# lanterndata/lantern

Hardware: AMD Instinct MI355X
Metric: QPS (recall@10 alongside), 1000000x768 f32 l2sq ef=64 k=10 (higher is better)
Workload: dtype f32

## Files before the change

include/lantern_gpu.h:

```cpp
#ifndef LANTERN_GPU_H
#define LANTERN_GPU_H

#include <stdbool.h>
#include <stddef.h>
#include <stdint.h>

#ifdef __cplusplus
extern "C" {
#endif

#define LANTERN_GPU_EXPORT __attribute__((visibility("default")))


typedef void       *usearch_index_t;
typedef uint64_t    usearch_key_t;
typedef uint64_t    usearch_label_t;
typedef float       usearch_distance_t;
typedef const char *usearch_error_t;

typedef enum usearch_metric_kind_t {
    usearch_metric_unknown_k = 0,
    usearch_metric_cos_k = 1,
    usearch_metric_l2sq_k = 3,
    usearch_metric_hamming_k = 8
// ... 186 lines not shown
LANTERN_GPU_EXPORT void lantern_gpu_last_filtered_each(usearch_index_t, uint32_t out[6], usearch_error_t *);
LANTERN_GPU_EXPORT void lantern_gpu_set_search_shape(usearch_index_t, int waves_per_query, int max_workgroups,
                                                     usearch_error_t *);

LANTERN_GPU_EXPORT void lantern_gpu_exact_search(usearch_index_t, const void *queries, size_t nq, size_t k,
                                                 uint32_t *slots, float *distances, usearch_error_t *);

LANTERN_GPU_EXPORT size_t lantern_gpu_dense_profile(int on, float *ms, uint32_t *rows, uint32_t *cols, uint32_t *fused, size_t cap);
LANTERN_GPU_EXPORT void lantern_gpu_exact_knn_stats(uint64_t *queries, uint64_t *certified, uint64_t *fallback);

LANTERN_GPU_EXPORT void lantern_gpu_search_row_trace(usearch_index_t, int on, size_t nq, size_t per_query_cap, uint32_t *trace,
                                                     uint32_t *counts, usearch_error_t *);

LANTERN_GPU_EXPORT int lantern_gpu_last_search_grid(usearch_index_t, usearch_error_t *);
LANTERN_GPU_EXPORT const char *lantern_gpu_plan_search(const int64_t in[31], uint32_t out[12]);

LANTERN_GPU_EXPORT void lantern_gpu_distance_gather(usearch_index_t, const void *query, const uint32_t *slots,
                                                    size_t n, float *out, usearch_error_t *);
LANTERN_GPU_EXPORT float lantern_gpu_last_gather_ms(usearch_index_t, usearch_error_t *);
LANTERN_GPU_EXPORT void lantern_gpu_search_screen_stats(usearch_index_t, uint64_t *logical, uint64_t *exact, usearch_error_t *);
LANTERN_GPU_EXPORT size_t lantern_gpu_export_screen(usearch_index_t, size_t first, size_t count, int8_t *rows, float *meta, float *norms,
                                                    usearch_error_t *);
LANTERN_GPU_EXPORT void lantern_gpu_screen_probe(usearch_index_t, const void *query, const uint32_t *slots, size_t n, float radius,
                                                 int workgroup, uint8_t *rejected, usearch_error_t *);
LANTERN_GPU_EXPORT void lantern_gpu_distance_matrix(const void *a, size_t na, const void *b, size_t nb,
                                                    usearch_scalar_kind_t, size_t dims, usearch_metric_kind_t,
                                                    int exact_order, float *out, usearch_error_t *);

LANTERN_GPU_EXPORT void lantern_gpu_assign_to_clusters(const float *dataset, size_t n, size_t row_dims, size_t subvector_start,
                                                       size_t subvector_dim, const float *centers, size_t k,
// ... 168 lines not shown
```

lantern_amd/capi.py:

```python
from __future__ import annotations

import ctypes as C
import os

import numpy as np

HERE = os.path.dirname(os.path.abspath(__file__))
LIB_PATH = os.path.join(HERE, "lib", "liblantern_gpu.so")

METRIC_COS, METRIC_L2SQ, METRIC_HAMMING = 1, 3, 8
SCALAR_F32, SCALAR_F16, SCALAR_I8, SCALAR_B1 = 1, 3, 4, 5
METRICS = {"cos": METRIC_COS, "l2sq": METRIC_L2SQ, "hamming": METRIC_HAMMING}
EMPTY = 0xFFFFFFFF
USEARCH_HEADER_SIZE = 136


class LanternGpuError(RuntimeError):
    pass


class InitOptions(C.Structure):
    _fields_ = [
        ("metric_kind", C.c_int),
        ("metric", C.c_void_p),
# ... 53 lines not shown
    "lantern_gpu_version", "lantern_gpu_device_count",
    "lantern_gpu_set_seed", "lantern_gpu_set_add_batch", "lantern_gpu_add_many", "lantern_gpu_flush",
    "lantern_gpu_add_with_level", "lantern_gpu_search_batch", "lantern_gpu_search_batch_device", "lantern_gpu_search_batch_device_strided",
    "lantern_gpu_set_search_shape", "lantern_gpu_exact_search", "lantern_gpu_dense_profile", "lantern_gpu_exact_knn_stats", "lantern_gpu_distance_gather",
    "lantern_gpu_host_alloc", "lantern_gpu_host_free", "lantern_gpu_save_stream", "lantern_gpu_pq_compact", "lantern_gpu_pq_expand", "lantern_gpu_memory_usage", "lantern_gpu_spec_profile", "lantern_gpu_search_unique_rows", "lantern_gpu_search_row_trace", "lantern_gpu_last_search_grid", "lantern_gpu_last_gather_ms", "lantern_gpu_search_screen_stats",
    "lantern_gpu_distance_matrix", "lantern_gpu_assign_to_clusters", "lantern_gpu_graph_info_get", "lantern_gpu_export_graph", "lantern_gpu_import_graph",
    "lantern_gpu_export_codes",
    "lantern_gpu_counters_get", "lantern_gpu_set_profiling", "lantern_gpu_build_profile_get", "lantern_gpu_search_phase_profile", "lantern_scan_begin", "lantern_scan_rescan", "lantern_scan_gettuple", "lantern_scan_trace", "lantern_scan_end",
    "lantern_l2sq_dist", "lantern_cos_dist", "lantern_hamming_dist", "lantern_index_server_start", "lantern_index_server_start_tls",
    "lantern_index_server_port", "lantern_index_server_status_port", "lantern_index_server_status",
    "lantern_index_server_served", "lantern_index_server_stop",
    "lantern_gpu_graph_checksum", "lantern_gpu_comm_unique_id", "lantern_gpu_comm_init_rccl", "lantern_gpu_comm_init_host",
    "lantern_gpu_comm_init_local", "lantern_gpu_comm_free", "lantern_gpu_comm_rank", "lantern_gpu_comm_world",
    "lantern_gpu_comm_set_timeout", "lantern_gpu_comm_stats", "lantern_gpu_comm_allgatherv_host",
    "lantern_gpu_comm_allgatherv_device", "lantern_gpu_shard_range", "lantern_gpu_add_sharded", "lantern_gpu_add_row_sharded", "lantern_gpu_search_partitioned", "lantern_gpu_search_batch_lane", "lantern_gpu_search_batch_lane_notify", "lantern_gpu_row_bytes",
    "lantern_gpu_level_for", "lantern_gpu_plan_batch", "lantern_gpu_row_shard_plan", "lantern_gpu_plan_search",
    "lantern_scan_server_start", "lantern_scan_server_start_fn", "lantern_scan_server_port", "lantern_scan_server_stats",
    "lantern_scan_server_batch_histogram", "lantern_scan_server_timing", "lantern_scan_server_stop", "lantern_scan_client_connect", "lantern_scan_client_search", "lantern_scan_client_search_next",
    "lantern_scan_client_close", "lantern_scan_begin_client",
    "lantern_mirror_acquire", "lantern_mirror_index", "lantern_mirror_version", "lantern_mirror_rebind", "lantern_mirror_advance", "lantern_mirror_release",
    "lantern_mirror_invalidate", "lantern_mirror_set_capacity", "lantern_mirror_stats",
    "UsearchNodeBytes", "usearch_init_node", "node_tuple_size", "label_from_node", "level_from_node", "reset_node_label", "get_node_neighbors_mut",
    "lantern_quant_bits_scalar_kind",
    "lantern_gpu_filter_from_labels", "lantern_gpu_filter_from_slot_bitmap", "lantern_gpu_filter_count", "lantern_gpu_filter_free",
    "lantern_gpu_set_filter_policy", "lantern_gpu_filter_stats", "lantern_gpu_last_filtered_launch", "lantern_gpu_search_batch_filtered", "lantern_gpu_search_batch_filtered_device",
    "lantern_gpu_cursor_search_filtered", "lantern_scan_set_filter",
    "lantern_gpu_filter_resident_bytes", "lantern_scan_server_start_filtered_fn", "lantern_scan_server_filter_stats", "lantern_scan_client_set_filter",
    "lantern_scan_client_clear_filter",
    "lantern_gpu_search_batch_filtered_each", "lantern_gpu_search_batch_filtered_each_device", "lantern_gpu_search_batch_filtered_each_lane", "lantern_gpu_last_filtered_each",
    "lantern_gpu_set_filter_seeds", "lantern_gpu_last_filtered_seeds",
    "lantern_gpu_search_batch_params", "lantern_gpu_search_batch_params_lane", "lantern_gpu_search_batch_params_lane_notify",
# ... 131 lines not shown
        "lantern_gpu_comm_world": (i32, [vp]),
        "lantern_gpu_comm_set_timeout": (None, [vp, C.c_double]),
        "lantern_gpu_comm_stats": (None, [vp, C.POINTER(u64), C.POINTER(u64)]),
        "lantern_gpu_comm_allgatherv_host": (None, [vp, vp, C.POINTER(sz), C.POINTER(sz), err]),
        "lantern_gpu_comm_allgatherv_device": (None, [vp, vp, C.POINTER(sz), C.POINTER(sz), vp, err]),
        "lantern_gpu_shard_range": (None, [sz, i32, i32, C.POINTER(sz), C.POINTER(sz)]),
        "lantern_gpu_add_sharded": (None, [vp, vp, vp, vp, sz, i32, err]),
        "lantern_gpu_add_row_sharded": (None, [vp, vp, vp, vp, sz, i32, err]),
        "lantern_gpu_search_partitioned": (None, [vp, vp, vp, sz, i32, sz, sz, vp, vp, vp, err]),
        "lantern_gpu_row_bytes": (sz, [vp, err]),
        "lantern_gpu_search_batch_lane": (None, [vp, i32, vp, sz, i32, sz, sz, vp, vp, vp, err]),
        "lantern_gpu_search_batch_lane_notify": (None, [vp, i32, vp, sz, i32, sz, sz, vp, vp, vp, vp, vp, err]),
        "lantern_gpu_level_for": (i32, [u64, u64, u32]),
        "lantern_gpu_plan_batch": (sz, [sz, i32, vp, sz, sz, sz]),
        "lantern_gpu_plan_search": (C.c_char_p, [vp, vp]),
        "lantern_gpu_row_shard_plan": (sz, [vp, i32, u64, u32, sz, sz, vp, vp, vp, sz]),
        "lantern_scan_server_start": (vp, [vp, C.c_char_p, i32, sz, C.c_uint, err]),
        "lantern_scan_server_start_fn": (vp, [BATCH_SEARCH_FN, vp, sz, C.c_char_p, i32, sz, C.c_uint, err]),
        "lantern_scan_server_port": (i32, [vp]),
        "lantern_scan_server_stats": (None, [vp, C.POINTER(u64), C.POINTER(u64), C.POINTER(u64), C.POINTER(u64)]),
        "lantern_scan_server_batch_histogram": (sz, [vp, C.POINTER(u64), sz]),
        "lantern_scan_server_timing": (None, [vp, C.POINTER(C.c_double)]),
        "lantern_scan_server_stop": (None, [vp]),
        "lantern_scan_client_connect": (vp, [C.c_char_p, i32, err]),
        "lantern_scan_client_search": (sz, [vp, vp, sz, sz, sz, vp, vp, err]),
        "lantern_scan_client_search_next": (sz, [vp, vp, sz, sz, sz, vp, vp, err]),
        "lantern_scan_client_close": (None, [vp]),
        "lantern_scan_begin_client": (vp, [vp, sz, i32, i32, err]),
        "lantern_mirror_acquire": (vp, [u64, u64, C.POINTER(InitOptions), vp, vp, sz, err]),
        "lantern_mirror_index": (vp, [vp]),
# ... 781 lines not shown

def plan_batch(size: int, max_level: int, pending_levels, max_batch: int, min_ratio: int) -> int:
    lv = np.ascontiguousarray(pending_levels, dtype=np.int32)
    return int(lib().lantern_gpu_plan_batch(size, max_level, _ptr(lv), lv.size, max_batch, min_ratio))


PLAN_SEARCH_IN = ("chunks", "M", "M0", "mcode", "n", "ef_default", "num_cus", "pq_compact", "pqd_inv", "pq_S16", "search_vis_slots", "search_max_wg",
                  "phase_profile", "spec_profile", "nq", "k", "ef", "skip", "waves", "each", "max_expansion", "env_spec_set", "env_spec",
                  "env_adc_spec_set", "env_adc_spec", "env_pq_adc", "env_spec_waves", "env_lds_list", "env_wide_rows", "env_solo", "env_waves_per_cu")
PLAN_SEARCH_OUT = ("path", "spec", "expansion", "waves", "grid", "vis_slots", "lds", "spec_prefetch", "spec_cache", "wide_rows", "took_spec", "lds_list")


def plan_search(fields) -> tuple[dict, str | None]:
    vals = [fields[n] for n in PLAN_SEARCH_IN] if isinstance(fields, dict) else list(fields)
    assert len(vals) == len(PLAN_SEARCH_IN)
    a, out = np.asarray(vals, dtype=np.int64), np.zeros(len(PLAN_SEARCH_OUT), dtype=np.uint32)
    why = lib().lantern_gpu_plan_search(_ptr(a), _ptr(out))
    return dict(zip(PLAN_SEARCH_OUT, (int(x) for x in out))), (why.decode() if why else None)


def row_shard_plan(shard_sizes, seed: int, M: int, max_batch: int, min_ratio: int):
    sizes = np.ascontiguousarray(shard_sizes, dtype=np.uint64)
    world = int(sizes.size)
    n = int(lib().lantern_gpu_row_shard_plan(_ptr(sizes), world, seed, M, max_batch, min_ratio, None, None, None, 0))
    first, count = np.zeros(max(n, 1), dtype=np.uintp), np.zeros(max(n, 1), dtype=np.uintp)
    share = np.zeros((max(n, 1), world), dtype=np.uintp)
    lib().lantern_gpu_row_shard_plan(_ptr(sizes), world, seed, M, max_batch, min_ratio, _ptr(first), _ptr(count), _ptr(share), n)
    return [(int(first[t]), int(count[t]), [int(x) for x in share[t]]) for t in range(n)]


def shard_range(n: int, world: int, rank: int) -> tuple[int, int]:
    b, e = C.c_size_t(), C.c_size_t()
    lib().lantern_gpu_shard_range(n, world, rank, C.byref(b), C.byref(e))
# ... 363 lines not shown
```

lantern_amd/csrc/device_common.hpp:

```cpp
#pragma once
#include <hip/hip_runtime.h>
#include <stdint.h>

namespace lgpu {

constexpr uint32_t EMPTY = 0xFFFFFFFFu;
#ifndef LGPU_ROW_BLOCK
#define LGPU_ROW_BLOCK 3
#endif
#ifndef LGPU_ROW_BLOCK_COS
#define LGPU_ROW_BLOCK_COS 2
#endif
#ifndef LGPU_LIST_PREFETCH
#define LGPU_LIST_PREFETCH 1
#endif
#ifndef LGPU_ROW_BLOCK1
#define LGPU_ROW_BLOCK1 4
#endif
#ifndef LGPU_SCREEN
#define LGPU_SCREEN 1
#endif

constexpr int M_COS = 1;
constexpr int M_L2SQ = 3;
// ... 480 lines not shown
    int32_t         max_level;
    const uint4    *pq_centers;
    uint32_t        pq_cps;
    uint32_t        pq_C;
    uint32_t        pq_inv;
    uint32_t        pq_row_bytes;
    const uint4    *screen;
    const float2   *screen_meta;
    uint32_t        screen_chunks;
};

__host__ __device__ __forceinline__ float screen_val(float s, uint32_t w, int b) { return s * (float)(int)(int8_t)(uint8_t)(w >> (8 * b)); }
__host__ __device__ inline bool screen_rows_for(uint32_t chunks) { return chunks >= 128; }
__host__ __device__ inline bool screen_cos_norm_ok(float r) { return r >= 0x1p-48f && r <= 0x1p48f; }
__host__ __device__ inline uint32_t screen_chunks_for(uint32_t chunks) { return (chunks + 3) / 4; }

__device__ __forceinline__ const uint4 *row_of(const View &v, uint32_t slot) { return v.vec + (size_t)slot * v.chunks; }

struct PqdRow
{
    const uint8_t *codes;
    const uint4   *centers;
    uint32_t       cps, C, inv;
    __device__ __forceinline__ uint4 operator[](int ch) const
    {
        const uint32_t sv = ((uint32_t)ch * inv) >> 16, off = (uint32_t)ch - sv * cps;
        const uint32_t code = codes[ sv ];
        return centers[ ((size_t)sv * C + code) * cps + off ];
    }
};
// ... 23 lines not shown
```

lantern_amd/csrc/index.hpp:

```cpp
#pragma once
#include <hip/hip_runtime.h>

#include <deque>
#include <mutex>
#include <string>
#include <thread>
#include <unordered_map>
#include <unordered_set>
#include <functional>
#include <vector>

#include "../../include/lantern_gpu.h"
#include "kernels.hpp"

namespace lgpu {

struct Cursor
{
    std::unordered_set<uint32_t> seen;
};

constexpr int kIndexLanes = 8;

enum ScratchSlot : int
// ... 199 lines not shown
uint32_t    vis_undo_cap();
int         search_grid(const Index *ix, size_t nq, int waves, int waves_per_cu);
int         search_grid(int num_cus, int max_wg, int forced_waves_per_cu, size_t nq, int waves, int waves_per_cu);
struct SearchEnv
{
    bool spec_set = false, adc_spec_set = false;
    int  spec = 0, spec_waves = 0, wide_rows = -1, waves_per_cu = 0;
    bool adc_spec = false, pq_adc = false, lds_list = false, solo = false;
};
SearchEnv search_env();
struct SearchPlanIn
{
    uint32_t  chunks = 0, M = 0, M0 = 0, ef_default = 0, pqd_inv = 0, pq_S16 = 0;
    int       mcode = 0, num_cus = 0, search_vis_slots = -1, search_max_wg = 0;
    bool      pq_compact = false, phase_profile = false, spec_profile = false;
    size_t    n = 0, nq = 0, k = 0, ef = 0, skip = 0;
    int       waves = 0;
    bool      each = false;
    uint32_t  max_expansion = 0;
    SearchEnv env;
};
enum SearchPath : uint32_t { kSearchAdc, kSearchPqd, kSearchClassic, kSearchSpec1, kSearchSpec2, kSearchTwin, kSearchSolo };
struct SearchPlan
{
    SearchPath  path = kSearchClassic;
    int         spec = 0, waves = 0, grid = 0, wide_rows = 0, lds_list = 0;
    uint32_t    expansion = 0, vis_slots = 0, spec_prefetch = 0, spec_cache = 0;
    size_t      lds = 0;
    bool        took_spec = false;
    const char *refusal = nullptr;
};
SearchPlan   plan_search(const SearchPlanIn &in);
SearchPlanIn search_plan_in(const Index *ix, size_t nq, size_t k, size_t ef, size_t skip, int waves);
struct EachLaunch
{
    const char *h_table = nullptr;
    size_t      table_bytes = 0;
    const char *d_table = nullptr;
    size_t      list_at = 0;
};
bool        run_search_device(Index *ix, const uint4 *d_queries, size_t nq, size_t k, size_t ef, size_t skip, const SearchOut &out,
                              hipStream_t stream, int waves, uint32_t *done = nullptr, uint32_t *done_flags = nullptr);
std::string params_check(const lantern_gpu_query_params *params, size_t nq, size_t k_stride);
// ... 30 lines not shown
```

lantern_amd/csrc/screen_probe_kernel.hip:

```cpp
#include "query_frame.hpp"

namespace lgpu {

constexpr uint32_t kProbeSlots = 64;

template <int METRIC>
__global__ void __launch_bounds__(512) k_screen_probe(View v, const uint4 *query, const uint32_t *slots, uint32_t n, float radius, uint8_t *out)
{
    constexpr int G = 64;
    const int     tid = threadIdx.x, T = blockDim.x;
    WalkLds       s;
    (void)carve_walk(lgpu_smem, s, v.chunks, kProbeSlots, kProbeSlots);
    if(tid == 0) {
        uint64_t *const sp = (uint64_t *)&s.scal[ S_SCREEN ];
        sp[ 0 ] = (uint64_t)v.screen;
        sp[ 1 ] = (uint64_t)v.screen_meta;
        s.scal[ S_NREJ ] = 0;
        s.scal[ S_NSURV ] = 0;
        s.scal[ S_QN2 ] = 0;
    }
    for(uint32_t i = tid; i < n; i += T) {
        s.newids[ i ] = slots[ i ];
        s.newkeys[ i ] = 0;
    }
    frame_stage<METRIC, G>(tid, T, s, query, 0, v.chunks);
    const float qn2 = __int_as_float(s.scal[ S_QN2 ]);
    (void)hop_distances_screened<METRIC, G, 2>(v, s, (int)n, make_key(radius, 0u), qn2);
    for(uint32_t i = tid; i < n; i += T) out[ i ] = s.newkeys[ i ] == ~0ull ? 1 : 0;
}

hipError_t launch_screen_probe(int metric, const View &v, const uint4 *query, const uint32_t *slots, uint32_t n, float radius, int threads,
                               uint8_t *out, hipStream_t stream)
{
    if(n == 0) return hipSuccess;
    if(n > kProbeSlots || (threads != 256 && threads != 512) || !v.screen || !v.screen_meta || !screen_rows_for(v.chunks)) return hipErrorInvalidValue;
    const size_t lds = walk_lds_bytes(v.chunks, kProbeSlots, kProbeSlots);
    if(metric == M_L2SQ) hipLaunchKernelGGL(k_screen_probe<M_L2SQ>, dim3(1), dim3(threads), lds, stream, v, query, slots, n, radius, out);
    else if(metric == M_COS) hipLaunchKernelGGL(k_screen_probe<M_COS>, dim3(1), dim3(threads), lds, stream, v, query, slots, n, radius, out);
    else return hipErrorInvalidValue;
    return hipGetLastError();
}

}
```

lantern_amd/csrc/search_kernel.hpp:

```cpp
#pragma once
#include <algorithm>
#include <cstddef>
#include <cstdlib>

#include "kernels.hpp"
#include "walk.hpp"
#include "walk_spec.hpp"
#ifndef LGPU_EXPERIMENTAL
#define LGPU_EXPERIMENTAL 0
#endif
#if LGPU_EXPERIMENTAL
#include "experimental/walk_twin.hpp"
#endif
#include "dispatch.hpp"
#include "query_frame.hpp"

namespace lgpu {

#define LGPU_SEARCH_ARG(base, field) LGPU_KARG(base, decltype(SearchArgs::field), offsetof(SearchArgs, field))
#define LGPU_VIEW_ARG(base, STRUCT, field) LGPU_KARG(base, decltype(View::field), offsetof(STRUCT, view) + offsetof(View, field))
#define LGPU_LOAD_VIEW(v, base, STRUCT)             \
    {                                               \
        v.vec = LGPU_VIEW_ARG(base, STRUCT, vec);   \
        v.chunks = LGPU_VIEW_ARG(base, STRUCT, chunks); \
// ... 59 lines not shown
            View               v;
            LGPU_LOAD_VIEW(v, ka, SearchArgs)
            if constexpr(METRIC >= M_PQD) LGPU_LOAD_VIEW_PQD(v, ka, SearchArgs)
            if constexpr(SCREEN) {
                if(tid == 0) {
                    uint64_t *const sp = (uint64_t *)&s.scal[ S_SCREEN ];
                    sp[ 0 ] = (uint64_t)LGPU_VIEW_ARG(ka, SearchArgs, screen);
                    sp[ 1 ] = (uint64_t)LGPU_VIEW_ARG(ka, SearchArgs, screen_meta);
                    s.scal[ S_NREJ ] = 0;
                }
            }
            uint32_t        bm_words;
            uint32_t *const bitmap = frame_bind<SearchArgs>(ka, s, bm_words);
            const int       ef = EACH ? (int)each.ef : (int)LGPU_SEARCH_ARG(ka, ef);
            frame_stage<METRIC, G>(tid, T, s, LGPU_FRAME_ARG(ka, SearchArgs, queries), q, v.chunks);
            if constexpr(PROF) {
                t_q = (unsigned long long)clock64();
                s.touched = LGPU_SEARCH_ARG(ka, touched);
                s.trace_cap = LGPU_SEARCH_ARG(ka, trace_cap);
                uint32_t *const tr = LGPU_SEARCH_ARG(ka, trace);
                s.trace = tr ? tr + (size_t)q * s.trace_cap : nullptr;
                s.trace_count = tr ? LGPU_SEARCH_ARG(ka, trace_count) + q : nullptr;
            }
            if(v.n != 0 && (!EACH || each.k != 0)) {
                uint32_t start;
                if constexpr(SPEC != 0) start = greedy_descent_spec<METRIC, G>(v, s, v.entry, v.max_level, 0, D);
                else start = greedy_descent<METRIC, G, PROF>(v, s, v.entry, v.max_level, 0, D);
                if constexpr(PROF) pc[ 6 ] = (unsigned long long)clock64() - t_q;
#if LGPU_EXPERIMENTAL
                if constexpr(SPEC == 3)
// ... 29 lines not shown
```

lantern_amd/csrc/search_launch.hpp:

```cpp
#pragma once
#include "search_kernel.hpp"

namespace lgpu {

#define LGPU_LAUNCH_SEARCH(...)                                                                                        \
    {                                                                                                                  \
        static LdsAttrCache attr_;        \
        ensure_dynamic_lds((const void *)k_search<__VA_ARGS__>, lds, attr_);    \
        hipLaunchKernelGGL((k_search<__VA_ARGS__>), dim3(grid), dim3(64 * waves), lds, stream, a);                     \
    }
#define LGPU_LAUNCH_SEARCH_KPL(MM, GG, PP, RR)                           \
    {                                                                    \
        if(kpl == 1) LGPU_LAUNCH_SEARCH(MM, GG, PP, RR, 1, 0, EACH)      \
        else if(kpl == 2) LGPU_LAUNCH_SEARCH(MM, GG, PP, RR, 2, 0, EACH) \
        else LGPU_LAUNCH_SEARCH(MM, GG, PP, RR, 0, 0, EACH)              \
    }

template <bool EACH> static hipError_t launch_search_classic(int metric, const SearchArgs &a, int waves, int grid, hipStream_t stream)
{
    if(EACH && a.phase_cycles) return hipErrorInvalidValue;
    const size_t lds = search_lds_bytes(a.view.chunks, a.ef, a.view.M0, a.frame.vis_slots);
    const int    kpl = a.lds_list ? 0 : a.ef <= 64 ? 1 : a.ef <= 128 ? 2 : 0;
    const int    G_ = group_lanes_for(a.view.chunks);
    if(a.wide_rows && !a.phase_cycles && G_ == 64) {
        bool launched = true;
        switch(metric) {
            case M_L2SQ: LGPU_LAUNCH_SEARCH_KPL(M_L2SQ, 64, false, 4); break;
            case M_COS: LGPU_LAUNCH_SEARCH_KPL(M_COS, 64, false, 4); break;
            case M_HAMMING: LGPU_LAUNCH_SEARCH_KPL(M_HAMMING, 64, false, 4); break;
            case M_L2SQ_F16: LGPU_LAUNCH_SEARCH_KPL(M_L2SQ_F16, 64, false, 4); break;
            case M_COS_F16: LGPU_LAUNCH_SEARCH_KPL(M_COS_F16, 64, false, 4); break;
            case M_L2SQ_PQD: LGPU_LAUNCH_SEARCH_KPL(M_L2SQ_PQD, 64, false, 4); break;
            case M_COS_PQD: LGPU_LAUNCH_SEARCH_KPL(M_COS_PQD, 64, false, 4); break;
            default: launched = false;
        }
        if(launched) return hipGetLastError();
// ... 72 lines not shown
```

lantern_amd/csrc/search_plan.cpp:

```cpp
#include "index.hpp"

#include <algorithm>
#include <cstdlib>
#include <cstring>

namespace lgpu {

SearchEnv search_env()
{
    SearchEnv e;
    if(const char *se = std::getenv("LANTERN_GPU_SPEC")) { e.spec_set = true; e.spec = std::atoi(se); }
    if(const char *se = std::getenv("LANTERN_GPU_ADC_SPEC")) { e.adc_spec_set = true; e.adc_spec = std::atoi(se) != 0; }
    if(const char *pa = std::getenv("LANTERN_GPU_PQ_ADC")) e.pq_adc = std::atoi(pa) != 0;
    if(const char *sw = std::getenv("LANTERN_GPU_SPEC_WAVES")) e.spec_waves = std::atoi(sw);
    if(const char *ll = std::getenv("LANTERN_GPU_LDS_LIST")) e.lds_list = std::atoi(ll) != 0;
    static const int  wide_env = std::getenv("LANTERN_GPU_WIDE_ROWS") ? std::atoi(std::getenv("LANTERN_GPU_WIDE_ROWS")) : -1;
    static const bool solo_auto = std::getenv("LANTERN_GPU_SOLO") && std::atoi(std::getenv("LANTERN_GPU_SOLO")) != 0;
    static const int  forced = std::getenv("LANTERN_GPU_WAVES_PER_CU") ? std::atoi(std::getenv("LANTERN_GPU_WAVES_PER_CU")) : 0;
    e.wide_rows = wide_env, e.solo = solo_auto, e.waves_per_cu = forced;
    return e;
}

SearchPlanIn search_plan_in(const Index *ix, size_t nq, size_t k, size_t ef, size_t skip, int waves)
{
    SearchPlanIn in;
    in.chunks = ix->chunks; in.M = ix->M; in.M0 = ix->M0; in.ef_default = ix->ef;
    in.mcode = ix->mcode; in.n = ix->n; in.num_cus = ix->num_cus;
    in.pq_compact = ix->pq_compact; in.pqd_inv = ix->pqd_inv; in.pq_S16 = ix->pq_S16;
    in.search_vis_slots = ix->search_vis_slots; in.search_max_wg = ix->search_max_wg;
    in.phase_profile = ix->phase_profile; in.spec_profile = ix->spec_profile;
    in.nq = nq; in.k = k; in.ef = ef; in.skip = skip; in.waves = waves;
    in.env = search_env();
    return in;
}

SearchPlan plan_search(const SearchPlanIn &in)
{
    const SearchEnv &env = in.env;
    const size_t     nq = in.nq;
    int              waves = in.waves;
    SearchPlan       p;
    size_t expansion = in.ef ? in.ef : in.ef_default;
    if(expansion < in.k + in.skip) expansion = in.k + in.skip;
    if(in.each) expansion = in.max_expansion;
    p.expansion = (uint32_t)expansion;
// ... 60 lines not shown
                    return p;
                }
            }
            if(spec == 3 && !(expansion <= 64 && (in.mcode == M_L2SQ || in.mcode == M_COS) && (group_lanes_for(in.chunks) == 64 || (in.mcode == M_L2SQ && group_lanes_for(in.chunks) == 16))))
                spec = 2;
#endif
        }
        waves = spec >= 2 ? 11 : spec == 1 ? 4 : waves < 0 ? -waves : 4;
        if(spec && env.spec_waves >= (spec >= 2 ? 4 : 2) && env.spec_waves <= (spec >= 2 ? 11 : 8)) waves = env.spec_waves;
    }
    const int      G_ = group_lanes_for(in.chunks), LW_ = G_ >= 32 ? 1 : G_ == 16 ? 2 : 4;
    const uint32_t spec_prefetch = spec && in.M0 % (uint32_t)LW_ == 0 && in.M0 <= (uint32_t)(G_ * LW_) ? 1u : 0u;
    const uint32_t spec_cache = !spec_prefetch ? 0u : spec >= 2 ? 128u : 64u;
    const size_t   spec_lds = spec ? search_spec_lds_bytes(in.M0, spec_prefetch, spec_cache, spec == 3) : 0;
    const size_t lds_budget = spec >= 2 ? 96 * 1024 : spec == 1 ? 39 * 1024 : 26 * 1024;
    uint32_t vis_slots = 1024;
    while(vis_slots < 8192 && vis_slots / 4 * 3 < expansion * in.M0 * 2) vis_slots <<= 1;
    if(in.search_vis_slots >= 0) vis_slots = (uint32_t)in.search_vis_slots / 4 * 4;
    while(vis_slots && search_lds_bytes(in.chunks, (uint32_t)expansion, in.M0, vis_slots) + spec_lds > lds_budget)
        vis_slots = vis_slots > 256 ? vis_slots - 256 : 0;
    if(vis_slots && vis_slots < 4 * in.M0) vis_slots = 0;
    p.lds = search_lds_bytes(in.chunks, (uint32_t)expansion, in.M0, vis_slots) + spec_lds;
    if(p.lds > 160 * 1024) { p.refusal = "lantern_gpu: ef/k exceed the 160 KiB LDS budget of the search kernel"; return p; }
    p.path = pqd ? kSearchPqd : spec == 0 ? kSearchClassic : spec == 1 ? kSearchSpec1 : spec == 2 ? kSearchSpec2 : kSearchTwin;
    p.spec = spec, p.took_spec = spec != 0;
    p.waves = waves, p.grid = search_grid(in.num_cus, in.search_max_wg, env.waves_per_cu, nq, waves, spec >= 2 ? waves : spec == 1 ? 16 : 24);
    p.vis_slots = vis_slots, p.spec_prefetch = spec_prefetch, p.spec_cache = spec_cache;
    p.wide_rows = spec ? 0 : env.wide_rows >= 0 ? env.wide_rows : (nq * (size_t)waves <= (size_t)in.num_cus * 16 && nq >= 64);
    return p;
}

static bool search_launch(Index *ix, const SearchPlan &p, const uint4 *d_queries, size_t nq, size_t k, size_t skip, const SearchOut &out,
                          hipStream_t stream, uint32_t *done, uint32_t *done_flags, const EachLaunch *each)
{
    const bool adc = p.path == kSearchAdc, pqd = p.path == kSearchPqd, solo = p.path == kSearchSolo;
    ix->last_search_grid = p.grid;
    const int slot = acquire_search_slot(ix, stream, (size_t)p.grid);
// ... 2 lines not shown
    a.view = ix->view();
    a.frame.queries = d_queries;
    a.frame.nq = (uint32_t)nq, a.k = (uint32_t)k, a.ef = p.expansion, a.skip = (uint32_t)skip;
    a.frame.labels = ix->d_labels;
    a.frame.out_labels = out.labels, a.frame.out_dists = out.dists, a.frame.out_slots = out.slots;
    a.frame.out_counts = out.counts, a.frame.out_D = out.D, a.frame.out_E = out.E;
    if(!solo) a.frame.bitmaps = ix->slot_bitmaps[ slot ], a.frame.bm_words = (uint32_t)ix->slot_words[ slot ], a.frame.undo_cap = vis_undo_cap();
    a.frame.vis_slots = p.vis_slots;
    a.frame.totals = ix->d_totals;
    a.screen_totals = ix->d_screen ? ix->d_totals + 48 : nullptr;
    a.frame.ticket = next_ticket(ix, nq, p.grid, stream);
    a.done = done, a.done_flags = done_flags;
    a.lds_list = p.lds_list, a.wide_rows = p.wide_rows;
    a.spec = p.spec, a.spec_prefetch = p.spec_prefetch, a.spec_cache = p.spec_cache;
    hipError_t e = hipSuccess;
    if(adc || pqd) a.view.vec = (const uint4 *)ix->d_codes16;
    if(adc) {
        a.view.chunks = ix->pq_S16 / 16;
        a.adc_centers = ix->d_centers;
        a.adc_S = ix->pq_S, a.adc_C = ix->pq_C, a.adc_subdim = ix->pq_subdim, a.adc_qchunks = ix->chunks;
    } else {
        if(pqd) {
            a.view.pq_centers = (const uint4 *)ix->d_centers;
            a.view.pq_cps = ix->pq_subdim / 4;
            a.view.pq_C = ix->pq_C;
            a.view.pq_inv = ix->pqd_inv;
            a.view.pq_row_bytes = ix->pq_S16;
        }
        const bool prof_walk = ix->phase_profile && !pqd && !each;
        a.phase_cycles = each ? nullptr : p.spec ? (ix->spec_profile ? ix->d_totals + 16 : nullptr) : prof_walk ? ix->d_totals + 8 : nullptr;
// ... 96 lines not shown
        at += cls[ c ].size();
    }
    for(int c = 0; c < 3; ++c) {
        if(cls[ c ].empty()) continue;
        if(!search_launch(ix, plans[ c ], d_queries, cls[ c ].size(), k_stride, 0, out, stream, nullptr, done_flags, &each[ c ])) return false;
        launches += 1;
        any_spec |= plans[ c ].took_spec ? 1u : 0u;
    }
    const uint32_t shape[ 6 ] = { launches, (uint32_t)cls[ 0 ].size(), (uint32_t)cls[ 1 ].size(), (uint32_t)cls[ 2 ].size(), std::max(top[ 0 ], std::max(top[ 1 ], top[ 2 ])), any_spec };
    std::copy(std::begin(shape), std::end(shape), ix->last_params);
    return true;
}

}

extern "C" const char *lantern_gpu_plan_search(const int64_t in[ 31 ], uint32_t out[ 12 ])
{
    if(!in || !out) return "lantern_gpu: null array";
    lgpu::SearchPlanIn s;
    s.chunks = (uint32_t)in[ 0 ]; s.M = (uint32_t)in[ 1 ]; s.M0 = (uint32_t)in[ 2 ]; s.mcode = (int)in[ 3 ]; s.n = (size_t)in[ 4 ];
    s.ef_default = (uint32_t)in[ 5 ]; s.num_cus = (int)in[ 6 ]; s.pq_compact = in[ 7 ] != 0; s.pqd_inv = (uint32_t)in[ 8 ]; s.pq_S16 = (uint32_t)in[ 9 ];
    s.search_vis_slots = (int)in[ 10 ]; s.search_max_wg = (int)in[ 11 ]; s.phase_profile = in[ 12 ] != 0; s.spec_profile = in[ 13 ] != 0;
    s.nq = (size_t)in[ 14 ]; s.k = (size_t)in[ 15 ]; s.ef = (size_t)in[ 16 ]; s.skip = (size_t)in[ 17 ]; s.waves = (int)in[ 18 ];
    s.each = in[ 19 ] != 0; s.max_expansion = (uint32_t)in[ 20 ];
    s.env.spec_set = in[ 21 ] != 0; s.env.spec = (int)in[ 22 ]; s.env.adc_spec_set = in[ 23 ] != 0; s.env.adc_spec = in[ 24 ] != 0;
    s.env.pq_adc = in[ 25 ] != 0; s.env.spec_waves = (int)in[ 26 ]; s.env.lds_list = in[ 27 ] != 0; s.env.wide_rows = (int)in[ 28 ];
    s.env.solo = in[ 29 ] != 0; s.env.waves_per_cu = (int)in[ 30 ];
    const lgpu::SearchPlan p = lgpu::plan_search(s);
    const uint32_t flat[ 12 ] = { (uint32_t)p.path, (uint32_t)p.spec, p.expansion, (uint32_t)p.waves, (uint32_t)p.grid, p.vis_slots, (uint32_t)p.lds,
                                  p.spec_prefetch, p.spec_cache, (uint32_t)p.wide_rows, p.took_spec ? 1u : 0u, (uint32_t)p.lds_list };
    std::copy(std::begin(flat), std::end(flat), out);
    return p.refusal;
}
```

lantern_amd/csrc/walk.hpp:

```cpp
#pragma once
#include <type_traits>

#include "device_common.hpp"

namespace lgpu {

enum { S_POS = 0, S_NNEW, S_CNT, S_ANY, S_BAD, S_CUR, S_CURD, S_CHANGED, S_VISCNT, S_SPILL, S_QN2, S_NNEW0, S_NNEW1, S_ANY0, S_ANY1,
       S_FRONT = 16, S_WORST = 20,
       S_MASK = 24,
       S_SCALARS = 28,
       S_NSURV = S_ANY0, S_NREJ = S_ANY1, S_SCREEN = S_MASK };

struct WalkLds
{
    uint4    *q;
    uint64_t *keys;
    uint64_t *keys2;
    uint64_t *newkeys;
    uint64_t *sorted;
    uint32_t *newids;
    int      *scal;
    uint32_t *vis;
    uint32_t  vis_slots;
    uint32_t *touched;
// ... 317 lines not shown
        if(gl == G - 1) {
            reread();
            uint64_t k0 = make_key(d0, id0);
            s.newkeys[ at(i) ] = k0;
            bool any = k0 < worst;
            if(j < nnew) {
                uint64_t k1 = make_key(d1, id1);
                s.newkeys[ at(j) ] = k1;
                any |= k1 < worst;
            }
            if(ANY && any) *any_slot = 1;
        }
    }
}

template <int METRIC, int G, int ROWS>
__device__ __forceinline__ int hop_distances_screened(const View &v, WalkLds &s, int nnew, uint64_t worst, float qn2)
{
    static_assert(METRIC == M_L2SQ || METRIC == M_COS, "the screen serves the f32 l2sq and cosine walks");
    constexpr int GS = 8, NB = 3;
    static_assert(G % GS == 0, "a screen group lies within one wave");
    const int       tid = threadIdx.x, T = blockDim.x, gs = tid / GS, gsl = tid % GS, NGS = T / GS;
    uint32_t *const surv = (uint32_t *)s.sorted;
    typedef uint32_t u32x4 __attribute__((ext_vector_type(4)));
    typedef float    f32x2 __attribute__((ext_vector_type(2)));
    typedef const __attribute__((address_space(1))) u32x4 *ScreenRow;
    typedef const __attribute__((address_space(1))) f32x2 *ScreenMeta;
    auto uniform = [](uint64_t x) {
        return (uint64_t)(uint32_t)__builtin_amdgcn_readfirstlane((int)(uint32_t)x) |
               (uint64_t)(uint32_t)__builtin_amdgcn_readfirstlane((int)(uint32_t)(x >> 32)) << 32;
    };
    const ScreenRow  screen = (ScreenRow)uniform(((const uint64_t *)&s.scal[ S_SCREEN ])[ 0 ]);
    const ScreenMeta screen_meta = (ScreenMeta)uniform(((const uint64_t *)&s.scal[ S_SCREEN ])[ 1 ]);
    const uint32_t   chunks = v.chunks, sch = screen_chunks_for(chunks);
    for(int j = gs; j < nnew; j += NGS) {
        const uint32_t id = s.newids[ j ];
        const ScreenRow row = screen + (size_t)id * sch;
        const f32x2     meta = screen_meta[ id ];
        float          acc = 0.f;
        for(uint32_t base = (uint32_t)gsl; base < sch; base += NB * GS) {
            u32x4 y[ NB ];
#pragma unroll
            for(int c = 0; c < NB; ++c)
                if(base + c * GS < sch) y[ c ] = row[ base + c * GS ];
#pragma unroll
            for(int c = 0; c < NB; ++c)
                if(base + c * GS < sch) {
                    const uint32_t w[ 4 ] = { y[ c ].x, y[ c ].y, y[ c ].z, y[ c ].w };
#pragma unroll
                    for(int k = 0; k < 4; ++k) {
                        const uint32_t qc = 4 * (base + c * GS) + (uint32_t)k;
                        const uint4    x = qc < chunks ? s.q[ qc ] : make_uint4(0u, 0u, 0u, 0u);
                        const float    xs[ 4 ] = { __uint_as_float(x.x), __uint_as_float(x.y), __uint_as_float(x.z), __uint_as_float(x.w) };
#pragma unroll
                        for(int b = 0; b < 4; ++b) {
                            if constexpr(METRIC == M_COS) {
                                acc = __builtin_fmaf(xs[ b ], (float)(int)(int8_t)(uint8_t)(w[ k ] >> (8 * b)), acc);
                            } else {
                                const float t = xs[ b ] - screen_val(meta.x, w[ k ], b);
                                acc = __builtin_fmaf(t, t, acc);
                            }
                        }
                    }
                }
        }
        acc = group_sum<GS>(acc);
        if(gsl == GS - 1) {
            bool reject = false;
            if constexpr(METRIC == M_COS) {
                const float rd = key_dist(worst), e = fmaxf(0x1p-12f, (float)(2 * chunks + 64) * 0x1p-24f);
                if(screen_cos_norm_ok(qn2)) {
                    const float sim8 = (acc * meta.x) / qn2;
                    const float ub = (sim8 + meta.y) + e;
                    reject = (1.f - ub) - e > rd;
                }
            } else {
                const float rd = key_dist(worst), ome = 1.f - fmaxf(0x1p-12f, (float)(2 * chunks + 64) * 0x1p-24f);
                if(__builtin_isfinite(acc)) {
                    const float a = __builtin_sqrtf(acc) * ome - meta.y;
                    const float lb = a > 0.f ? a * a : 0.f;
                    reject = lb > 0x1p-100f && lb * ome > rd;
                }
            }
            if(reject) s.newkeys[ j ] = ~0ull;
            else surv[ atomicAdd(&s.scal[ S_NSURV ], 1) ] = (uint32_t)j;
        }
    }
    __syncthreads();
    const int ns = s.scal[ S_NSURV ];
    if(tid == 0) s.scal[ S_NREJ ] += nnew - ns;
    return ns;
}

template <int METRIC, int G, bool PROF = false, int ROWS = 2>
__device__ int search_level(const View &v, WalkLds &s, uint32_t *bitmap, uint32_t bm_words, uint32_t start, int level, int ef,
                            uint32_t &D, uint32_t &E, unsigned long long *prof = nullptr)
// ... 434 lines not shown
```

Baseline: 2.297 million.

## Quantize query to int16 planes for integer dot4 screen distance bounds

The f32 query is quantized once per search into hi/lo int8 planes stored in extra LDS, together with a scale, an error bound and the quantized norm. The int8 screen pass then computes the distance bound with integer dot4 instructions instead of per-byte float FMAs, widening the bound by the quantization error so it stays conservative. The search planner reserves the extra LDS, which can shrink the visited-slot table, and it turns screening off for configurations it does not support.

```diff
diff --git a/include/lantern_gpu.h b/include/lantern_gpu.h
--- a/include/lantern_gpu.h
+++ b/include/lantern_gpu.h
@@ -224,6 +224,7 @@
 
 LANTERN_GPU_EXPORT int lantern_gpu_last_search_grid(usearch_index_t, usearch_error_t *);
 LANTERN_GPU_EXPORT const char *lantern_gpu_plan_search(const int64_t in[31], uint32_t out[12]);
+LANTERN_GPU_EXPORT const char *lantern_gpu_plan_search_screen(const int64_t in[32], uint32_t out[13]);
 
 LANTERN_GPU_EXPORT void lantern_gpu_distance_gather(usearch_index_t, const void *query, const uint32_t *slots,
                                                     size_t n, float *out, usearch_error_t *);
diff --git a/lantern_amd/capi.py b/lantern_amd/capi.py
--- a/lantern_amd/capi.py
+++ b/lantern_amd/capi.py
@@ -91,7 +91,7 @@
     "lantern_gpu_comm_init_local", "lantern_gpu_comm_free", "lantern_gpu_comm_rank", "lantern_gpu_comm_world",
     "lantern_gpu_comm_set_timeout", "lantern_gpu_comm_stats", "lantern_gpu_comm_allgatherv_host",
     "lantern_gpu_comm_allgatherv_device", "lantern_gpu_shard_range", "lantern_gpu_add_sharded", "lantern_gpu_add_row_sharded", "lantern_gpu_search_partitioned", "lantern_gpu_search_batch_lane", "lantern_gpu_search_batch_lane_notify", "lantern_gpu_row_bytes",
-    "lantern_gpu_level_for", "lantern_gpu_plan_batch", "lantern_gpu_row_shard_plan", "lantern_gpu_plan_search",
+    "lantern_gpu_level_for", "lantern_gpu_plan_batch", "lantern_gpu_row_shard_plan", "lantern_gpu_plan_search", "lantern_gpu_plan_search_screen",
     "lantern_scan_server_start", "lantern_scan_server_start_fn", "lantern_scan_server_port", "lantern_scan_server_stats",
     "lantern_scan_server_batch_histogram", "lantern_scan_server_timing", "lantern_scan_server_stop", "lantern_scan_client_connect", "lantern_scan_client_search", "lantern_scan_client_search_next",
     "lantern_scan_client_close", "lantern_scan_begin_client",
@@ -253,6 +253,7 @@
         "lantern_gpu_level_for": (i32, [u64, u64, u32]),
         "lantern_gpu_plan_batch": (sz, [sz, i32, vp, sz, sz, sz]),
         "lantern_gpu_plan_search": (C.c_char_p, [vp, vp]),
+        "lantern_gpu_plan_search_screen": (C.c_char_p, [vp, vp]),
         "lantern_gpu_row_shard_plan": (sz, [vp, i32, u64, u32, sz, sz, vp, vp, vp, sz]),
         "lantern_scan_server_start": (vp, [vp, C.c_char_p, i32, sz, C.c_uint, err]),
         "lantern_scan_server_start_fn": (vp, [BATCH_SEARCH_FN, vp, sz, C.c_char_p, i32, sz, C.c_uint, err]),
@@ -1064,9 +1065,15 @@
 def plan_search(fields) -> tuple[dict, str | None]:
     vals = [fields[n] for n in PLAN_SEARCH_IN] if isinstance(fields, dict) else list(fields)
     assert len(vals) == len(PLAN_SEARCH_IN)
-    a, out = np.asarray(vals, dtype=np.int64), np.zeros(len(PLAN_SEARCH_OUT), dtype=np.uint32)
-    why = lib().lantern_gpu_plan_search(_ptr(a), _ptr(out))
-    return dict(zip(PLAN_SEARCH_OUT, (int(x) for x in out))), (why.decode() if why else None)
+    if isinstance(fields, dict) and "screen" in fields:
+        names = PLAN_SEARCH_OUT + ("screen_lds",)
+        a, out = np.asarray(vals + [fields["screen"]], dtype=np.int64), np.zeros(len(names), dtype=np.uint32)
+        why = lib().lantern_gpu_plan_search_screen(_ptr(a), _ptr(out))
+    else:
+        names = PLAN_SEARCH_OUT
+        a, out = np.asarray(vals, dtype=np.int64), np.zeros(len(names), dtype=np.uint32)
+        why = lib().lantern_gpu_plan_search(_ptr(a), _ptr(out))
+    return dict(zip(names, (int(x) for x in out))), (why.decode() if why else None)
 
 
 def row_shard_plan(shard_sizes, seed: int, M: int, max_batch: int, min_ratio: int):
diff --git a/lantern_amd/csrc/device_common.hpp b/lantern_amd/csrc/device_common.hpp
--- a/lantern_amd/csrc/device_common.hpp
+++ b/lantern_amd/csrc/device_common.hpp
@@ -518,6 +518,8 @@
 __host__ __device__ inline bool screen_rows_for(uint32_t chunks) { return chunks >= 128; }
 __host__ __device__ inline bool screen_cos_norm_ok(float r) { return r >= 0x1p-48f && r <= 0x1p48f; }
 __host__ __device__ inline uint32_t screen_chunks_for(uint32_t chunks) { return (chunks + 3) / 4; }
+__host__ __device__ inline uint32_t screen_query_lds_bytes(uint32_t chunks) { return 16 + screen_chunks_for(chunks) * 32; }
+__host__ __device__ inline bool screen_l2_scale_ok(float s) { return s >= 0x1p-40f && s <= 0x1p40f; }
 
 __device__ __forceinline__ const uint4 *row_of(const View &v, uint32_t slot) { return v.vec + (size_t)slot * v.chunks; }
 
diff --git a/lantern_amd/csrc/index.hpp b/lantern_amd/csrc/index.hpp
--- a/lantern_amd/csrc/index.hpp
+++ b/lantern_amd/csrc/index.hpp
@@ -237,6 +237,7 @@
     uint32_t  chunks = 0, M = 0, M0 = 0, ef_default = 0, pqd_inv = 0, pq_S16 = 0;
     int       mcode = 0, num_cus = 0, search_vis_slots = -1, search_max_wg = 0;
     bool      pq_compact = false, phase_profile = false, spec_profile = false;
+    bool      screen = false;
     size_t    n = 0, nq = 0, k = 0, ef = 0, skip = 0;
     int       waves = 0;
     bool      each = false;
@@ -250,6 +251,7 @@
     int         spec = 0, waves = 0, grid = 0, wide_rows = 0, lds_list = 0;
     uint32_t    expansion = 0, vis_slots = 0, spec_prefetch = 0, spec_cache = 0;
     size_t      lds = 0;
+    uint32_t    screen_lds = 0;
     bool        took_spec = false;
     const char *refusal = nullptr;
 };
diff --git a/lantern_amd/csrc/screen_probe_kernel.hip b/lantern_amd/csrc/screen_probe_kernel.hip
--- a/lantern_amd/csrc/screen_probe_kernel.hip
+++ b/lantern_amd/csrc/screen_probe_kernel.hip
@@ -25,6 +25,7 @@
     }
     frame_stage<METRIC, G>(tid, T, s, query, 0, v.chunks);
     const float qn2 = __int_as_float(s.scal[ S_QN2 ]);
+    screen_stage_query<METRIC>(tid, s, v.chunks, qn2);
     (void)hop_distances_screened<METRIC, G, 2>(v, s, (int)n, make_key(radius, 0u), qn2);
     for(uint32_t i = tid; i < n; i += T) out[ i ] = s.newkeys[ i ] == ~0ull ? 1 : 0;
 }
@@ -34,7 +35,7 @@
 {
     if(n == 0) return hipSuccess;
     if(n > kProbeSlots || (threads != 256 && threads != 512) || !v.screen || !v.screen_meta || !screen_rows_for(v.chunks)) return hipErrorInvalidValue;
-    const size_t lds = walk_lds_bytes(v.chunks, kProbeSlots, kProbeSlots);
+    const size_t lds = walk_lds_bytes(v.chunks, kProbeSlots, kProbeSlots) + screen_query_lds_bytes(v.chunks);
     if(metric == M_L2SQ) hipLaunchKernelGGL(k_screen_probe<M_L2SQ>, dim3(1), dim3(threads), lds, stream, v, query, slots, n, radius, out);
     else if(metric == M_COS) hipLaunchKernelGGL(k_screen_probe<M_COS>, dim3(1), dim3(threads), lds, stream, v, query, slots, n, radius, out);
     else return hipErrorInvalidValue;
diff --git a/lantern_amd/csrc/search_kernel.hpp b/lantern_amd/csrc/search_kernel.hpp
--- a/lantern_amd/csrc/search_kernel.hpp
+++ b/lantern_amd/csrc/search_kernel.hpp
@@ -97,6 +97,9 @@
             uint32_t *const bitmap = frame_bind<SearchArgs>(ka, s, bm_words);
             const int       ef = EACH ? (int)each.ef : (int)LGPU_SEARCH_ARG(ka, ef);
             frame_stage<METRIC, G>(tid, T, s, LGPU_FRAME_ARG(ka, SearchArgs, queries), q, v.chunks);
+            if constexpr(SCREEN) {
+                if(LGPU_VIEW_ARG(ka, SearchArgs, screen)) screen_stage_query<METRIC>(tid, s, v.chunks, __int_as_float(s.scal[ S_QN2 ]));
+            }
             if constexpr(PROF) {
                 t_q = (unsigned long long)clock64();
                 s.touched = LGPU_SEARCH_ARG(ka, touched);
diff --git a/lantern_amd/csrc/search_launch.hpp b/lantern_amd/csrc/search_launch.hpp
--- a/lantern_amd/csrc/search_launch.hpp
+++ b/lantern_amd/csrc/search_launch.hpp
@@ -19,7 +19,7 @@
 template <bool EACH> static hipError_t launch_search_classic(int metric, const SearchArgs &a, int waves, int grid, hipStream_t stream)
 {
     if(EACH && a.phase_cycles) return hipErrorInvalidValue;
-    const size_t lds = search_lds_bytes(a.view.chunks, a.ef, a.view.M0, a.frame.vis_slots);
+    const size_t lds = search_lds_bytes(a.view.chunks, a.ef, a.view.M0, a.frame.vis_slots) + (a.view.screen ? screen_query_lds_bytes(a.view.chunks) : 0);
     const int    kpl = a.lds_list ? 0 : a.ef <= 64 ? 1 : a.ef <= 128 ? 2 : 0;
     const int    G_ = group_lanes_for(a.view.chunks);
     if(a.wide_rows && !a.phase_cycles && G_ == 64) {
diff --git a/lantern_amd/csrc/search_plan.cpp b/lantern_amd/csrc/search_plan.cpp
--- a/lantern_amd/csrc/search_plan.cpp
+++ b/lantern_amd/csrc/search_plan.cpp
@@ -29,6 +29,7 @@
     in.pq_compact = ix->pq_compact; in.pqd_inv = ix->pqd_inv; in.pq_S16 = ix->pq_S16;
     in.search_vis_slots = ix->search_vis_slots; in.search_max_wg = ix->search_max_wg;
     in.phase_profile = ix->phase_profile; in.spec_profile = ix->spec_profile;
+    in.screen = ix->d_screen && ix->d_screen_meta;
     in.nq = nq; in.k = k; in.ef = ef; in.skip = skip; in.waves = waves;
     in.env = search_env();
     return in;
@@ -119,13 +120,17 @@
     const uint32_t spec_cache = !spec_prefetch ? 0u : spec >= 2 ? 128u : 64u;
     const size_t   spec_lds = spec ? search_spec_lds_bytes(in.M0, spec_prefetch, spec_cache, spec == 3) : 0;
     const size_t lds_budget = spec >= 2 ? 96 * 1024 : spec == 1 ? 39 * 1024 : 26 * 1024;
+    const bool   screened = in.screen && spec == 0 && !pqd && screen_rows_for(in.chunks) && (in.mcode == M_L2SQ || in.mcode == M_COS) &&
+                          !(in.phase_profile && !in.each) && !env.lds_list && expansion <= 128;
+    const size_t screen_lds = screened ? screen_query_lds_bytes(in.chunks) : 0;
     uint32_t vis_slots = 1024;
     while(vis_slots < 8192 && vis_slots / 4 * 3 < expansion * in.M0 * 2) vis_slots <<= 1;
     if(in.search_vis_slots >= 0) vis_slots = (uint32_t)in.search_vis_slots / 4 * 4;
-    while(vis_slots && search_lds_bytes(in.chunks, (uint32_t)expansion, in.M0, vis_slots) + spec_lds > lds_budget)
+    while(vis_slots && search_lds_bytes(in.chunks, (uint32_t)expansion, in.M0, vis_slots) + spec_lds + screen_lds > lds_budget)
         vis_slots = vis_slots > 256 ? vis_slots - 256 : 0;
     if(vis_slots && vis_slots < 4 * in.M0) vis_slots = 0;
-    p.lds = search_lds_bytes(in.chunks, (uint32_t)expansion, in.M0, vis_slots) + spec_lds;
+    p.lds = search_lds_bytes(in.chunks, (uint32_t)expansion, in.M0, vis_slots) + spec_lds + screen_lds;
+    p.screen_lds = (uint32_t)screen_lds;
     if(p.lds > 160 * 1024) { p.refusal = "lantern_gpu: ef/k exceed the 160 KiB LDS budget of the search kernel"; return p; }
     p.path = pqd ? kSearchPqd : spec == 0 ? kSearchClassic : spec == 1 ? kSearchSpec1 : spec == 2 ? kSearchSpec2 : kSearchTwin;
     p.spec = spec, p.took_spec = spec != 0;
@@ -158,6 +163,7 @@
     a.lds_list = p.lds_list, a.wide_rows = p.wide_rows;
     a.spec = p.spec, a.spec_prefetch = p.spec_prefetch, a.spec_cache = p.spec_cache;
     hipError_t e = hipSuccess;
+    if(!p.screen_lds) a.view.screen = nullptr, a.view.screen_meta = nullptr, a.view.screen_chunks = 0;
     if(adc || pqd) a.view.vec = (const uint4 *)ix->d_codes16;
     if(adc) {
         a.view.chunks = ix->pq_S16 / 16;
@@ -284,10 +290,11 @@
 
 }
 
-extern "C" const char *lantern_gpu_plan_search(const int64_t in[ 31 ], uint32_t out[ 12 ])
+static const char *plan_search_flat(const int64_t *in, bool screen, uint32_t *out, uint32_t *screen_lds)
 {
     if(!in || !out) return "lantern_gpu: null array";
     lgpu::SearchPlanIn s;
+    s.screen = screen;
     s.chunks = (uint32_t)in[ 0 ]; s.M = (uint32_t)in[ 1 ]; s.M0 = (uint32_t)in[ 2 ]; s.mcode = (int)in[ 3 ]; s.n = (size_t)in[ 4 ];
     s.ef_default = (uint32_t)in[ 5 ]; s.num_cus = (int)in[ 6 ]; s.pq_compact = in[ 7 ] != 0; s.pqd_inv = (uint32_t)in[ 8 ]; s.pq_S16 = (uint32_t)in[ 9 ];
     s.search_vis_slots = (int)in[ 10 ]; s.search_max_wg = (int)in[ 11 ]; s.phase_profile = in[ 12 ] != 0; s.spec_profile = in[ 13 ] != 0;
@@ -300,5 +307,12 @@
     const uint32_t flat[ 12 ] = { (uint32_t)p.path, (uint32_t)p.spec, p.expansion, (uint32_t)p.waves, (uint32_t)p.grid, p.vis_slots, (uint32_t)p.lds,
                                   p.spec_prefetch, p.spec_cache, (uint32_t)p.wide_rows, p.took_spec ? 1u : 0u, (uint32_t)p.lds_list };
     std::copy(std::begin(flat), std::end(flat), out);
+    if(screen_lds) *screen_lds = p.screen_lds;
     return p.refusal;
 }
+extern "C" const char *lantern_gpu_plan_search(const int64_t in[ 31 ], uint32_t out[ 12 ]) { return plan_search_flat(in, false, out, nullptr); }
+extern "C" const char *lantern_gpu_plan_search_screen(const int64_t in[ 32 ], uint32_t out[ 13 ])
+{
+    if(!in || !out) return "lantern_gpu: null array";
+    return plan_search_flat(in, in[ 31 ] != 0, out, out + 12);
+}
diff --git a/lantern_amd/csrc/walk.hpp b/lantern_amd/csrc/walk.hpp
--- a/lantern_amd/csrc/walk.hpp
+++ b/lantern_amd/csrc/walk.hpp
@@ -355,11 +355,70 @@
     }
 }
 
+
+__device__ __forceinline__ uint32_t *screen_query_block(const WalkLds &s) { return s.vis + s.vis_slots; }
+
+template <int METRIC> __device__ __forceinline__ void screen_stage_query(const int tid, const WalkLds &s, uint32_t chunks, float qn2)
+{
+    uint32_t *const blk = screen_query_block(s);
+    if(__builtin_amdgcn_readfirstlane(tid) < 64) {
+        const uint32_t lane = (uint32_t)tid, sch = screen_chunks_for(chunks);
+        uint32_t       mb = 0;
+        for(uint32_t i = lane; i < chunks; i += 64) {
+            const uint4 x = s.q[ i ];
+            mb = max(max(mb, x.x & 0x7FFFFFFFu), max(max(x.y & 0x7FFFFFFFu, x.z & 0x7FFFFFFFu), x.w & 0x7FFFFFFFu));
+        }
+        for(int off = 32; off > 0; off >>= 1) mb = max(mb, (uint32_t)__shfl_xor((int)mb, off));
+        const float sx = __uint_as_float(mb) / 32639.f;
+        const bool  ok = mb < 0x7F800000u && mb != 0u && (METRIC == M_COS ? (sx >= 0x1p-126f && sx <= 0x1p100f) : screen_l2_scale_ok(sx));
+        float    S = 0.f;
+        uint32_t hh = 0, hl = 0, ll = 0;
+        for(uint32_t i = lane; i < 4 * sch; i += 64) {
+            const uint4 x = i < chunks ? s.q[ i ] : make_uint4(0u, 0u, 0u, 0u);
+            const float xs[ 4 ] = { __uint_as_float(x.x), __uint_as_float(x.y), __uint_as_float(x.z), __uint_as_float(x.w) };
+            uint32_t    hw = 0, lw = 0;
+#pragma unroll
+            for(int b = 0; b < 4; ++b) {
+                const float q = ok ? xs[ b ] / sx : 0.f;
+                const float Xf = fminf(fmaxf(__builtin_rintf(q), -32639.f), 32639.f);
+                const float rho = __builtin_fabsf(q - Xf) + 0x1p-9f;
+                S = __builtin_fmaf(rho, rho, S);
+                const int X = (int)Xf, h = (X + 128) >> 8, l = X - 256 * h;
+                hw |= ((uint32_t)h & 0xFFu) << (8 * b);
+                lw |= ((uint32_t)l & 0xFFu) << (8 * b);
+            }
+            hh = (uint32_t)dot4_i8(hw, hw, (int)hh);
+            hl = (uint32_t)dot4_i8(hw, lw, (int)hl);
+            ll = (uint32_t)dot4_i8(lw, lw, (int)ll);
+            blk[ 4 + 8 * (i / 4) + i % 4 ] = hw;
+            blk[ 8 + 8 * (i / 4) + i % 4 ] = lw;
+        }
+        S = group_sum<64>(S);
+        hh = group_sum<64>(hh), hl = group_sum<64>(hl), ll = group_sum<64>(ll);
+        if(lane == 63) {
+            float delta = __builtin_inff(), nx2 = 0.f;
+            if(ok) {
+                delta = (sx * __builtin_sqrtf(S)) * (1.f + 0x1p-10f);
+                if constexpr(METRIC == M_COS) delta = (delta / qn2) * (1.f + 0x1p-10f);
+                nx2 = (sx * sx) * (float)(65536.0 * (double)(int)hh + 512.0 * (double)(int)hl + (double)(int)ll);
+            }
+            blk[ 0 ] = __float_as_uint(ok ? sx : 0.f);
+            blk[ 1 ] = __float_as_uint(delta);
+            blk[ 2 ] = __float_as_uint(nx2);
+            blk[ 3 ] = 0u;
+        }
+    }
+    __syncthreads();
+}
+
+#ifndef LGPU_SCREEN_NB
+#define LGPU_SCREEN_NB 3
+#endif
 template <int METRIC, int G, int ROWS>
 __device__ __forceinline__ int hop_distances_screened(const View &v, WalkLds &s, int nnew, uint64_t worst, float qn2)
 {
     static_assert(METRIC == M_L2SQ || METRIC == M_COS, "the screen serves the f32 l2sq and cosine walks");
-    constexpr int GS = 8, NB = 3;
+    constexpr int GS = 8, NB = LGPU_SCREEN_NB;
     static_assert(G % GS == 0, "a screen group lies within one wave");
     const int       tid = threadIdx.x, T = blockDim.x, gs = tid / GS, gsl = tid % GS, NGS = T / GS;
     uint32_t *const surv = (uint32_t *)s.sorted;
@@ -374,11 +433,13 @@
     const ScreenRow  screen = (ScreenRow)uniform(((const uint64_t *)&s.scal[ S_SCREEN ])[ 0 ]);
     const ScreenMeta screen_meta = (ScreenMeta)uniform(((const uint64_t *)&s.scal[ S_SCREEN ])[ 1 ]);
     const uint32_t   chunks = v.chunks, sch = screen_chunks_for(chunks);
+    const uint32_t *const blk = screen_query_block(s);
+    const uint4 *const    planes = (const uint4 *)(blk + 4);
     for(int j = gs; j < nnew; j += NGS) {
         const uint32_t id = s.newids[ j ];
         const ScreenRow row = screen + (size_t)id * sch;
         const f32x2     meta = screen_meta[ id ];
-        float          acc = 0.f;
+        int            ih = 0, il = 0, c2 = 0;
         for(uint32_t base = (uint32_t)gsl; base < sch; base += NB * GS) {
             u32x4 y[ NB ];
 #pragma unroll
@@ -387,40 +448,42 @@
 #pragma unroll
             for(int c = 0; c < NB; ++c)
                 if(base + c * GS < sch) {
+                    const uint4    hq = planes[ 2 * (base + c * GS) ], lq = planes[ 2 * (base + c * GS) + 1 ];
                     const uint32_t w[ 4 ] = { y[ c ].x, y[ c ].y, y[ c ].z, y[ c ].w };
+                    const uint32_t hs[ 4 ] = { hq.x, hq.y, hq.z, hq.w }, ls[ 4 ] = { lq.x, lq.y, lq.z, lq.w };
 #pragma unroll
                     for(int k = 0; k < 4; ++k) {
-                        const uint32_t qc = 4 * (base + c * GS) + (uint32_t)k;
-                        const uint4    x = qc < chunks ? s.q[ qc ] : make_uint4(0u, 0u, 0u, 0u);
-                        const float    xs[ 4 ] = { __uint_as_float(x.x), __uint_as_float(x.y), __uint_as_float(x.z), __uint_as_float(x.w) };
-#pragma unroll
-                        for(int b = 0; b < 4; ++b) {
-                            if constexpr(METRIC == M_COS) {
-                                acc = __builtin_fmaf(xs[ b ], (float)(int)(int8_t)(uint8_t)(w[ k ] >> (8 * b)), acc);
-                            } else {
-                                const float t = xs[ b ] - screen_val(meta.x, w[ k ], b);
-                                acc = __builtin_fmaf(t, t, acc);
-                            }
-                        }
-                    }
-                }
-        }
-        acc = group_sum<GS>(acc);
+                        ih = dot4_i8(hs[ k ], w[ k ], ih);
+                        il = dot4_i8(ls[ k ], w[ k ], il);
+                        if constexpr(METRIC == M_L2SQ) c2 = dot4_i8(w[ k ], w[ k ], c2);
+                    }
+                }
+        }
+        ih = (int)group_sum<GS>((uint32_t)ih);
+        il = (int)group_sum<GS>((uint32_t)il);
+        if constexpr(METRIC == M_L2SQ) c2 = (int)group_sum<GS>((uint32_t)c2);
         if(gsl == GS - 1) {
-            bool reject = false;
+            bool        reject = false;
+            const float sx = __uint_as_float(blk[ 0 ]), delta = __uint_as_float(blk[ 1 ]);
+            const float fI = (float)(256.0 * (double)ih + (double)il);
+            const float rd = key_dist(worst), e = fmaxf(0x1p-12f, (float)(2 * chunks + 64) * 0x1p-24f);
             if constexpr(METRIC == M_COS) {
-                const float rd = key_dist(worst), e = fmaxf(0x1p-12f, (float)(2 * chunks + 64) * 0x1p-24f);
                 if(screen_cos_norm_ok(qn2)) {
-                    const float sim8 = (acc * meta.x) / qn2;
-                    const float ub = (sim8 + meta.y) + e;
+                    const float sim8 = ((fI * sx) * meta.x) / qn2;
+                    const float ub = ((sim8 + meta.y * (1.f + delta)) + delta) + e;
                     reject = (1.f - ub) - e > rd;
                 }
             } else {
-                const float rd = key_dist(worst), ome = 1.f - fmaxf(0x1p-12f, (float)(2 * chunks + 64) * 0x1p-24f);
-                if(__builtin_isfinite(acc)) {
-                    const float a = __builtin_sqrtf(acc) * ome - meta.y;
-                    const float lb = a > 0.f ? a * a : 0.f;
-                    reject = lb > 0x1p-100f && lb * ome > rd;
+                const float ome = 1.f - e;
+                if(screen_l2_scale_ok(meta.x)) {
+                    const float nx2 = __uint_as_float(blk[ 2 ]);
+                    const float R = (2.f * (sx * meta.x)) * fI, Q = (meta.x * meta.x) * (float)c2;
+                    const float m = ((nx2 - R) + Q) - 0x1p-20f * (nx2 + Q);
+                    if(__builtin_isfinite(m)) {
+                        const float a = (__builtin_sqrtf(fmaxf(m, 0.f)) * ome - meta.y) - delta;
+                        const float lb = a > 0.f ? a * a : 0.f;
+                        reject = lb > 0x1p-100f && lb * ome > rd;
+                    }
                 }
             }
             if(reject) s.newkeys[ j ] = ~0ull;
```

Result: faster. 2.422 million (median of 6 runs) (+5.4%).
